# regicide211212/multi-style-transfer-gan

Hardware: AMD Instinct MI355X
Metric: train-step images/sec (fwd+bwd+loss), 256x256 batch32 (higher is better)
Workload: dtype f32; 1 GPU; config 3: reference CycleGAN train_step (2x EnhancedGenerator + 2x EnhancedDiscriminator, channels=16, num_transformer_blocks=0), 32 image pairs/GPU at 256x256, fwd+bwd+loss+Adam; per_gpu_batch=32, size=256, channels=16, parallelism=dp1, collective=none, losses_finite=True

## Files before the change

multi-style-transfer-gan_amd/mstg_hip/csrc/common.h:

```cpp
#pragma once
#include <hip/hip_runtime.h>
#include <stdint.h>
#include <stdio.h>
#include <string.h>

#include "mstg_hip.h"

typedef float f32x4 __attribute__((ext_vector_type(4)));
typedef float f32x2 __attribute__((ext_vector_type(2)));

namespace mstg {

extern thread_local char g_last_error[256];
inline int fail_launch(hipError_t e, const char* what) {
    snprintf(g_last_error, sizeof(g_last_error), "%s: %s", what, hipGetErrorString(e));
    return MSTG_E_LAUNCH;
}
inline int fail_arg(int code, const char* what) {
    snprintf(g_last_error, sizeof(g_last_error), "%s", what);
    return code;
}
#define MSTG_CHECK_LAUNCH(what)                                   \
    do {                                                          \
        hipError_t e__ = hipGetLastError();                       \
        if (e__ != hipSuccess) return mstg::fail_launch(e__, what); \
    } while (0)

extern bool g_prof_on;
void prof_begin(const void* host_fn, hipStream_t st);
void prof_end(hipStream_t st);
#define MSTG_LAUNCH(kern, grid, block, lds, st, ...)                               \
    do {                                                                           \
        const bool prof__ = mstg::g_prof_on;                                       \
        if (prof__) mstg::prof_begin((const void*)(kern), (hipStream_t)(st));      \
        hipLaunchKernelGGL(kern, grid, block, lds, st, __VA_ARGS__);               \
        if (prof__) mstg::prof_end((hipStream_t)(st));                             \
    } while (0)

extern thread_local bool t_ws_packed;
#define MSTG_PACK_LAUNCH(...)                      \
    do {                                           \
        if (!mstg::t_ws_packed) MSTG_LAUNCH(__VA_ARGS__); \
    } while (0)

enum EnvKnob {
    ENV_ATTN_BLK4, ENV_ATTN_BLK64, ENV_WGRAD_1X1, ENV_WGRAD_TS_MAXCH, ENV_WGRAD_PLAIN, ENV_WGRAD_OLD, ENV_NO_DPACK, ENV_IGEMM,
    ENV_STREAM, ENV_PF, ENV_WGLOB, ENV_HEAVY_PER_CU, ENV_DBG, ENV_DBG_LDS_KB, ENV_MS_WGRAD_PACKED, ENV_MS_FWD4, ENV_NO_PACK_CACHE,
    ENV_P32, ENV_P32_TH, ENV_P32_WLDS, ENV_P32_DBG, ENV_P32_OCC, ENV_ATTN_REG, ENV_NFW_ADAPT, ENV_BSUMS_ALL, ENV_ATTN_BIG32, ENV_NORM_WGS,
    ENV_CONV_IMG, ENV_COUNT
};
const char* env_get(EnvKnob k);

int cu_count();
struct OccCache {
    const void* kern = nullptr;
    size_t lds = 0;
    int occ = 1;
};
int persistent_occupancy(OccCache& c, const void* kern, size_t lds);

constexpr int WAVE = 64;

__device__ __forceinline__ f32x4 mfma16(float a, float b, f32x4 c) {
    return __builtin_amdgcn_mfma_f32_16x16x4f32(a, b, c, 0, 0, 0);
}

__device__ __forceinline__ float wave_sum(float v) {
#pragma unroll
    for (int o = 32; o > 0; o >>= 1) v += __shfl_xor(v, o, 64);
    return v;
}

__device__ __forceinline__ float apply_act(float v, int act) {
    switch (act) {
        case MSTG_ACT_RELU: return v > 0.f ? v : 0.f;
        case MSTG_ACT_LEAKY02: return v > 0.f ? v : 0.2f * v;
        case MSTG_ACT_TANH: return tanhf(v);
        case MSTG_ACT_GELU: return 0.5f * v * (1.f + erff(v * 0.70710678118654752f));
        default: return v;
    }
}
__device__ __forceinline__ float act_grad(float v, int act) {
    switch (act) {
        case MSTG_ACT_RELU: return v > 0.f ? 1.f : 0.f;
        case MSTG_ACT_LEAKY02: return v > 0.f ? 1.f : 0.2f;
        case MSTG_ACT_TANH: return 1.f - v * v;
        case MSTG_ACT_GELU: return 0.5f * (1.f + erff(v * 0.70710678118654752f)) + v * 0.3989422804014327f * expf(-0.5f * v * v);
        default: return 1.f;
    }
}

__device__ __forceinline__ int xcd_swizzle(int bid, int nblk) {
    const int q = nblk >> 3, r = nblk & 7, xcd = bid & 7, k = bid >> 3;
    return (xcd < r ? xcd * (q + 1) : r * (q + 1) + (xcd - r) * q) + k;
}


__host__ __device__ __forceinline__ unsigned magic_u32(unsigned d) { return 0xFFFFFFFFu / d + 1u; }

template <int NB>
__device__ __forceinline__ void stage_window_batch(const float* __restrict__ img, float* __restrict__ lds, int total, int e0, int cols,
                                                   int nq, unsigned m_cols, unsigned m_nq, int y0, int x0, int H, int W, int ctot,
                                                   int nq_valid, int ckp, int tid, int rowpad) {
    f32x4 v[NB];
    int dst[NB];
    bool ok[NB];
#pragma unroll
    for (int k = 0; k < NB; ++k) {
        const int e = e0 + 256 * k + tid;
        const int p = nq == 1 ? e : (int)__umulhi((unsigned)e, m_nq);
        const int q = e - p * nq;
        const int r = (int)__umulhi((unsigned)p, m_cols), c = p - r * cols;
        const int iy = y0 + r, ix = x0 + c;
        ok[k] = e < total && (unsigned)iy < (unsigned)H && (unsigned)ix < (unsigned)W && q < nq_valid;
        const unsigned off = ok[k] ? (unsigned)(iy * W + ix) * (unsigned)ctot + 4u * q : 0u;
        v[k] = *reinterpret_cast<const f32x4*>(img + off);
        dst[k] = e < total ? p * ckp + 4 * q + r * rowpad : -1;
    }
#pragma unroll
    for (int k = 0; k < NB; ++k)
        if (dst[k] >= 0) *reinterpret_cast<f32x4*>(&lds[dst[k]]) = ok[k] ? v[k] : f32x4{0.f, 0.f, 0.f, 0.f};
}

__device__ __forceinline__ void stage_window(const float* __restrict__ img, float* __restrict__ lds, int rows, int cols, int nq,
                                             unsigned m_cols, unsigned m_nq, int y0, int x0, int H, int W, int ctot, int nq_valid,
                                             int ckp, int tid, int rowpad = 0) {
    const int total = rows * cols * nq;
    int e0 = 0;
    for (; e0 + 1024 < total; e0 += 2048)
        stage_window_batch<8>(img, lds, total, e0, cols, nq, m_cols, m_nq, y0, x0, H, W, ctot, nq_valid, ckp, tid, rowpad);
    for (; e0 < total; e0 += 1024)
        stage_window_batch<4>(img, lds, total, e0, cols, nq, m_cols, m_nq, y0, x0, H, W, ctot, nq_valid, ckp, tid, rowpad);
}

__device__ __forceinline__ void stage_window_c4(const float* __restrict__ img, float* __restrict__ lds, int rows, int cols,
                                                unsigned m_cols, int y0, int x0, int H, int W, unsigned sy, unsigned sx, unsigned sc,
                                                int nch, int tid) {
    const int total = rows * cols;
    for (int e0 = 0; e0 < total; e0 += 1024) {
        f32x4 v[4];
        bool ok[4];
#pragma unroll
        for (int k = 0; k < 4; ++k) {
            const int e = e0 + 256 * k + tid;
            const int r = (int)__umulhi((unsigned)e, m_cols), c = e - r * cols;
            const int iy = y0 + r, ix = x0 + c;
            ok[k] = e < total && (unsigned)iy < (unsigned)H && (unsigned)ix < (unsigned)W;
            const unsigned off = ok[k] ? (unsigned)iy * sy + (unsigned)ix * sx : 0u;
#pragma unroll
            for (int ch = 0; ch < 4; ++ch) v[k][ch] = img[off + (ch < nch ? ch * sc : 0u)];
        }
#pragma unroll
        for (int k = 0; k < 4; ++k) {
            const int e = e0 + 256 * k + tid;
            if (e < total) {
                f32x4 w = {0.f, 0.f, 0.f, 0.f};
#pragma unroll
                for (int ch = 0; ch < 4; ++ch)
                    if (ok[k] && ch < nch) w[ch] = v[k][ch];
                *reinterpret_cast<f32x4*>(&lds[e * 4]) = w;
            }
        }
    }
}

inline int cdiv(int a, int b) { return (a + b - 1) / b; }
inline size_t cdivz(size_t a, size_t b) { return (a + b - 1) / b; }

}
```

multi-style-transfer-gan_amd/mstg_hip/csrc/norm.hip:

```cpp
#include "common.h"
#include <stdlib.h>

namespace mstg {

constexpr float NORM_EPS = 1e-5f;

struct NormGeom {
    int N, HW, C, split, chunk;
};

static NormGeom norm_geom(int N, int HW, int C) {
    NormGeom g;
    g.N = N; g.HW = HW; g.C = C;
    int wgs = 1024;
    { const char* e = env_get(ENV_NORM_WGS); if (e && atoi(e) >= 64) wgs = atoi(e); }
    int split = wgs / (N > 0 ? N : 1);
    if (split < 1) split = 1;
    const int maxsplit = cdiv(HW, 256);
    if (split > maxsplit) split = maxsplit;
    g.chunk = cdiv(HW, split);
    g.split = cdiv(HW, g.chunk);
    return g;
}

template <bool BWD>
__global__ __launch_bounds__(256) void norm_partial_kernel(const float* __restrict__ x, const float* __restrict__ dy,
                                                           const float* __restrict__ stats, const float* __restrict__ gamma,
                                                           const float* __restrict__ beta, float* __restrict__ partial,
                                                           NormGeom g, int act, int batch) {
    extern __shared__ __attribute__((aligned(16))) float red[];
    const int C = g.C, C4 = C >> 2, rows = 256 / C4;
    const int sp = blockIdx.x, n = blockIdx.y, tid = threadIdx.x;
    const int q = tid % C4, row = tid / C4;
    const int p0 = sp * g.chunk, p1 = min(g.HW, p0 + g.chunk);
    const float* xb = x + (size_t)n * g.HW * C;
    f32x4 s1 = {0.f, 0.f, 0.f, 0.f}, s2 = {0.f, 0.f, 0.f, 0.f};
    if (row < rows) {
        if (!BWD) {
            const f32x4 K = *reinterpret_cast<const f32x4*>((batch ? x : xb) + 4 * q);
            int p = p0 + row;
            constexpr int PX = 8;
            for (; p + (PX - 1) * rows < p1; p += PX * rows) {
                f32x4 v[PX];
#pragma unroll
                for (int k = 0; k < PX; ++k) v[k] = *reinterpret_cast<const f32x4*>(xb + (size_t)(p + k * rows) * C + 4 * q);
#pragma unroll
                for (int k = 0; k < PX; ++k) {
                    const f32x4 w = v[k] - K;
                    s1 += w;
                    s2 += w * w;
                }
            }
            for (; p < p1; p += rows) {
                const f32x4 v = *reinterpret_cast<const f32x4*>(xb + (size_t)p * C + 4 * q) - K;
                s1 += v;
                s2 += v * v;
            }
        } else {
            const float* st = stats + (size_t)(batch ? 0 : n) * C * 2;
            f32x4 mu, rs, ga = {1.f, 1.f, 1.f, 1.f}, be = {0.f, 0.f, 0.f, 0.f};
#pragma unroll
            for (int e = 0; e < 4; ++e) { mu[e] = st[(4 * q + e) * 2]; rs[e] = st[(4 * q + e) * 2 + 1]; }
            if (batch) { ga = *reinterpret_cast<const f32x4*>(gamma + 4 * q); be = *reinterpret_cast<const f32x4*>(beta + 4 * q); }
            const float* dyb = dy + (size_t)n * g.HW * C;
            int p = p0 + row;
            constexpr int PX = 8;
            for (; p + (PX - 1) * rows < p1; p += PX * rows) {
                f32x4 xv[PX], gv[PX];
#pragma unroll
                for (int k = 0; k < PX; ++k) {
                    xv[k] = *reinterpret_cast<const f32x4*>(xb + (size_t)(p + k * rows) * C + 4 * q);
                    gv[k] = *reinterpret_cast<const f32x4*>(dyb + (size_t)(p + k * rows) * C + 4 * q);
                }
#pragma unroll
                for (int k = 0; k < PX; ++k) {
                    const f32x4 xh = (xv[k] - mu) * rs;
                    f32x4 gg = gv[k];
#pragma unroll
                    for (int e = 0; e < 4; ++e) gg[e] *= act_grad(xh[e] * ga[e] + be[e], act);
                    s1 += gg;
                    s2 += gg * xh;
                }
            }
            for (; p < p1; p += rows) {
                const f32x4 xh = (*reinterpret_cast<const f32x4*>(xb + (size_t)p * C + 4 * q) - mu) * rs;
                f32x4 gg = *reinterpret_cast<const f32x4*>(dyb + (size_t)p * C + 4 * q);
#pragma unroll
                for (int e = 0; e < 4; ++e) gg[e] *= act_grad(xh[e] * ga[e] + be[e], act);
                s1 += gg;
                s2 += gg * xh;
            }
        }
        *reinterpret_cast<f32x4*>(&red[(row * 2 + 0) * C + 4 * q]) = s1;
        *reinterpret_cast<f32x4*>(&red[(row * 2 + 1) * C + 4 * q]) = s2;
    }
    __syncthreads();
    for (int e = tid; e < 2 * C; e += 256) {
        float acc = 0.f;
        for (int r = 0; r < rows; ++r) acc += red[r * 2 * C + e];
        partial[((size_t)n * g.split + sp) * 2 * C + e] = acc;
    }
}

template <bool BWD>
__global__ __launch_bounds__(256) void norm_apply_kernel(const float* __restrict__ x, const float* __restrict__ dy,
                                                         const float* __restrict__ residual, float* __restrict__ out,
                                                         float* __restrict__ stats, const float* __restrict__ gamma,
                                                         const float* __restrict__ beta, float* __restrict__ running_mean,
                                                         float* __restrict__ running_var, float* __restrict__ dgamma,
                                                         float* __restrict__ dbeta, const float* __restrict__ partial,
                                                         NormGeom g, int act, int batch, int psplit) {
    extern __shared__ __attribute__((aligned(16))) float sm[];
    const int C = g.C, C4 = C >> 2, rows = 256 / C4;
    const int sp = blockIdx.x, n = blockIdx.y, tid = threadIdx.x;
    const float cnt = batch ? (float)g.N * (float)g.HW : (float)g.HW;
    for (int c = tid; c < C; c += 256) {
        float t1 = 0.f, t2 = 0.f;
        if (batch != 2 && batch != 3) {
            const int nb = batch ? 0 : n, ne = batch ? g.N : n + 1;
            for (int nn = nb; nn < ne; ++nn) {
                const float* pp = partial + (size_t)nn * psplit * 2 * C + c;
                int s = 0;
                for (; s + 8 <= psplit; s += 8) {
                    float a[8], b[8];
#pragma unroll
                    for (int k = 0; k < 8; ++k) {
                        a[k] = pp[(size_t)(s + k) * 2 * C];
                        b[k] = pp[(size_t)(s + k) * 2 * C + C];
                    }
#pragma unroll
                    for (int k = 0; k < 8; ++k) {
                        t1 += a[k];
                        t2 += b[k];
                    }
                }
                for (; s < psplit; ++s) {
                    t1 += pp[(size_t)s * 2 * C];
                    t2 += pp[(size_t)s * 2 * C + C];
                }
            }
        }
        if (!BWD) {
            float mean, rstd;
            if (batch == 2) {
                mean = running_mean[c];
                rstd = rsqrtf(running_var[c] + NORM_EPS);
            } else if (batch == 3) {
                mean = stats[((size_t)n * C + c) * 2];
                rstd = stats[((size_t)n * C + c) * 2 + 1];
            } else {
                const float K = (batch ? x : x + (size_t)n * g.HW * C)[c];
                const float e1 = t1 / cnt;
                float var = t2 / cnt - e1 * e1;
                var = var > 0.f ? var : 0.f;
                mean = K + e1;
                rstd = rsqrtf(var + NORM_EPS);
                if (batch == 1 && sp == 0 && n == 0) {
                    running_mean[c] = 0.9f * running_mean[c] + 0.1f * mean;
                    running_var[c] = 0.9f * running_var[c] + 0.1f * var * (cnt / fmaxf(cnt - 1.f, 1.f));
                }
            }
            if (batch != 3 && sp == 0 && (!batch || n == 0)) {
                stats[((size_t)(batch ? 0 : n) * C + c) * 2] = mean;
                stats[((size_t)(batch ? 0 : n) * C + c) * 2 + 1] = rstd;
            }
            const bool affine = batch == 1 || batch == 2;
            const float ga = affine ? gamma[c] : 1.f, be = affine ? beta[c] : 0.f;
            sm[c] = rstd * ga;
            sm[C + c] = be;
            sm[2 * C + c] = mean;
        } else {
            const float* st = stats + (size_t)(batch ? 0 : n) * C * 2;
            const float mu = st[c * 2], rs = st[c * 2 + 1];
            const float ga = batch ? gamma[c] : 1.f;
            const float m1 = batch == 2 ? 0.f : t1 / cnt, m2 = batch == 2 ? 0.f : t2 / cnt;
            if (batch == 1 && sp == 0 && n == 0) { dgamma[c] = t2; dbeta[c] = t1; }
            sm[c] = mu;
            sm[C + c] = rs;
            sm[2 * C + c] = m1;
            sm[3 * C + c] = m2;
            (void)ga;
        }
    }
    __syncthreads();
    const int q = tid % C4, row = tid / C4;
    if (row >= rows) return;
    const int p0 = sp * g.chunk, p1 = min(g.HW, p0 + g.chunk);
    const size_t base = (size_t)n * g.HW * C;
    if (!BWD) {
        const f32x4 A = *reinterpret_cast<const f32x4*>(&sm[4 * q]), B = *reinterpret_cast<const f32x4*>(&sm[C + 4 * q]);
        const f32x4 M = *reinterpret_cast<const f32x4*>(&sm[2 * C + 4 * q]);
        int p = p0 + row;
        constexpr int PX = 8;
        for (; p + (PX - 1) * rows < p1; p += PX * rows) {
            f32x4 v[PX], r[PX];
#pragma unroll
            for (int k = 0; k < PX; ++k) {
                const size_t o = base + (size_t)(p + k * rows) * C + 4 * q;
                v[k] = __builtin_nontemporal_load(reinterpret_cast<const f32x4*>(x + o));
                if (residual) r[k] = __builtin_nontemporal_load(reinterpret_cast<const f32x4*>(residual + o));
            }
#pragma unroll
            for (int k = 0; k < PX; ++k) {
                const size_t o = base + (size_t)(p + k * rows) * C + 4 * q;
                f32x4 w = (v[k] - M) * A + B;
#pragma unroll
                for (int e = 0; e < 4; ++e) w[e] = apply_act(w[e], act);
                if (residual) w += r[k];
                *reinterpret_cast<f32x4*>(out + o) = w;
            }
        }
        for (; p < p1; p += rows) {
            const size_t o = base + (size_t)p * C + 4 * q;
            f32x4 v = (*reinterpret_cast<const f32x4*>(x + o) - M) * A + B;
#pragma unroll
            for (int e = 0; e < 4; ++e) v[e] = apply_act(v[e], act);
            if (residual) v += *reinterpret_cast<const f32x4*>(residual + o);
            *reinterpret_cast<f32x4*>(out + o) = v;
        }
    } else {
        const f32x4 mu = *reinterpret_cast<const f32x4*>(&sm[4 * q]), rs = *reinterpret_cast<const f32x4*>(&sm[C + 4 * q]);
        const f32x4 m1 = *reinterpret_cast<const f32x4*>(&sm[2 * C + 4 * q]), m2 = *reinterpret_cast<const f32x4*>(&sm[3 * C + 4 * q]);
        f32x4 ga = {1.f, 1.f, 1.f, 1.f}, be = {0.f, 0.f, 0.f, 0.f};
        if (batch) { ga = *reinterpret_cast<const f32x4*>(gamma + 4 * q); be = *reinterpret_cast<const f32x4*>(beta + 4 * q); }
        int p = p0 + row;
        constexpr int PX = 8;
        for (; p + (PX - 1) * rows < p1; p += PX * rows) {
            f32x4 xv[PX], gv[PX];
#pragma unroll
            for (int k = 0; k < PX; ++k) {
                const size_t o = base + (size_t)(p + k * rows) * C + 4 * q;
                xv[k] = __builtin_nontemporal_load(reinterpret_cast<const f32x4*>(x + o));
                gv[k] = __builtin_nontemporal_load(reinterpret_cast<const f32x4*>(dy + o));
            }
#pragma unroll
            for (int k = 0; k < PX; ++k) {
                const size_t o = base + (size_t)(p + k * rows) * C + 4 * q;
                const f32x4 xh = (xv[k] - mu) * rs;
                f32x4 gg = gv[k];
#pragma unroll
                for (int e = 0; e < 4; ++e) gg[e] *= act_grad(xh[e] * ga[e] + be[e], act);
                *reinterpret_cast<f32x4*>(out + o) = rs * ga * (gg - m1 - xh * m2);
            }
        }
        for (; p < p1; p += rows) {
            const size_t o = base + (size_t)p * C + 4 * q;
            const f32x4 xh = (*reinterpret_cast<const f32x4*>(x + o) - mu) * rs;
            f32x4 gg = *reinterpret_cast<const f32x4*>(dy + o);
#pragma unroll
            for (int e = 0; e < 4; ++e) gg[e] *= act_grad(xh[e] * ga[e] + be[e], act);
            *reinterpret_cast<f32x4*>(out + o) = rs * ga * (gg - m1 - xh * m2);
        }
    }
}

__device__ __forceinline__ void norm_row_sums(const float* __restrict__ partial, int n, int split, int C, int groups, float* red, float& t1,
                                              float& t2) {
    const int tid = threadIdx.x, c = tid % C, grp = tid / C;
    t1 = t2 = 0.f;
    if (grp < groups) {
        const float* pp = partial + (size_t)n * split * 2 * C + c;
        int s = grp;
        for (; s + 7 * groups < split; s += 8 * groups) {
            float a[8], b[8];
#pragma unroll
            for (int k = 0; k < 8; ++k) {
                a[k] = pp[(size_t)(s + k * groups) * 2 * C];
                b[k] = pp[(size_t)(s + k * groups) * 2 * C + C];
            }
#pragma unroll
            for (int k = 0; k < 8; ++k) {
                t1 += a[k];
                t2 += b[k];
            }
        }
        for (; s < split; s += groups) {
            t1 += pp[(size_t)s * 2 * C];
            t2 += pp[(size_t)s * 2 * C + C];
        }
    }
    if (groups > 1) {
        if (grp < groups) {
            red[(grp * 2 + 0) * C + c] = t1;
            red[(grp * 2 + 1) * C + c] = t2;
        }
        __syncthreads();
        if (grp == 0) {
            t1 = t2 = 0.f;
            for (int k = 0; k < groups; ++k) {
                t1 += red[(k * 2 + 0) * C + c];
                t2 += red[(k * 2 + 1) * C + c];
            }
        }
    }
}

static int norm_groups(const NormGeom& g) { return g.split > 32 && g.C <= 128 ? 256 / g.C : 1; }
static int norm_row_threads(const NormGeom& g) { const int t = g.C * norm_groups(g); return t < 64 ? 64 : ((t + 63) / 64) * 64; }

__global__ void norm_stats_kernel(const float* __restrict__ x, const float* __restrict__ partial, float* __restrict__ stats, NormGeom g,
                                  int groups) {
    extern __shared__ __attribute__((aligned(16))) float red[];
    const int n = blockIdx.x, C = g.C;
    const float cnt = (float)g.HW;
    float t1, t2;
    norm_row_sums(partial, n, g.split, C, groups, red, t1, t2);
    if ((int)threadIdx.x < C) {
        const int c = threadIdx.x;
        const float K = x[(size_t)n * g.HW * C + c];
        const float e1 = t1 / cnt;
        float var = t2 / cnt - e1 * e1;
        var = var > 0.f ? var : 0.f;
        stats[((size_t)n * C + c) * 2] = K + e1;
        stats[((size_t)n * C + c) * 2 + 1] = rsqrtf(var + NORM_EPS);
    }
}

__global__ void norm_sums_kernel(const float* __restrict__ partial, float* __restrict__ sums, NormGeom g, int groups) {
    extern __shared__ __attribute__((aligned(16))) float red[];
    const int n = blockIdx.x, C = g.C;
    float t1, t2;
    norm_row_sums(partial, n, g.split, C, groups, red, t1, t2);
    if ((int)threadIdx.x < C) {
        sums[((size_t)n * 2 + 0) * C + threadIdx.x] = t1;
        sums[((size_t)n * 2 + 1) * C + threadIdx.x] = t2;
    }
}

static int norm_check(int N, int HW, int C) {
    if (N <= 0 || HW <= 0 || C <= 0) return fail_arg(MSTG_E_BADARG, "norm: empty tensor");
    if (C % 4 || C > 1024) return fail_arg(MSTG_E_ALIGN, "norm: C must be a multiple of 4 and <= 1024");
    return MSTG_OK;
}

}

using namespace mstg;

extern "C" size_t mstg_norm_workspace_bytes(int N, int HW, int C) {
    if (N <= 0 || HW <= 0 || C <= 0) return 0;
    const NormGeom g = norm_geom(N, HW, C);
    return ((size_t)N * g.split * 2 * C + (size_t)N * 2 * C) * sizeof(float);
}

extern "C" int mstg_norm_act_fwd(const float* x, const float* residual, float* y, float* stats, int N, int HW, int C, int act,
                                 int batch_stats, const float* gamma, const float* beta, float* running_mean,
                                 float* running_var, void* workspace, size_t workspace_bytes, void* stream) {
    if (int rc = norm_check(N, HW, C)) return rc;
    if (!x || !y || !stats || !workspace) return fail_arg(MSTG_E_BADARG, "norm_fwd: null pointer");
    if (batch_stats && (!gamma || !beta || !running_mean || !running_var)) return fail_arg(MSTG_E_BADARG, "norm_fwd: batch norm needs gamma/beta/running stats");
    if (act == MSTG_ACT_TANH) return fail_arg(MSTG_E_UNSUPPORTED, "norm_fwd: tanh epilogue not supported");
    const NormGeom g = norm_geom(N, HW, C);
    if (workspace_bytes < mstg_norm_workspace_bytes(N, HW, C)) return fail_arg(MSTG_E_WORKSPACE, "norm_fwd: workspace too small");
    hipStream_t st = (hipStream_t)stream;
    const int rows = 256 / (C / 4);
    dim3 grid(g.split, N);
    if (batch_stats != 2) {
        MSTG_LAUNCH((norm_partial_kernel<false>), grid, dim3(256), (size_t)rows * 2 * C * sizeof(float), st, x, nullptr, nullptr,
                           gamma, beta, (float*)workspace, g, act, batch_stats);
        MSTG_CHECK_LAUNCH("norm_partial_kernel");
    }
    if (batch_stats == 0 && g.split > 32) {
        const int groups = norm_groups(g);
        MSTG_LAUNCH(norm_stats_kernel, dim3(N), dim3(norm_row_threads(g)), (size_t)groups * 2 * C * sizeof(float), st, x,
                    (const float*)workspace, stats, g, groups);
        MSTG_CHECK_LAUNCH("norm_stats_kernel");
        MSTG_LAUNCH((norm_apply_kernel<false>), grid, dim3(256), (size_t)4 * C * sizeof(float), st, x, nullptr, residual, y, stats, nullptr,
                    nullptr, nullptr, nullptr, nullptr, nullptr, nullptr, g, act, 3, 0);
        MSTG_CHECK_LAUNCH("norm_apply_kernel");
        return MSTG_OK;
    }
    MSTG_LAUNCH((norm_apply_kernel<false>), grid, dim3(256), (size_t)4 * C * sizeof(float), st, x, nullptr, residual, y, stats,
                       gamma, beta, running_mean, running_var, nullptr, nullptr, (const float*)workspace, g, act, batch_stats, g.split);
    MSTG_CHECK_LAUNCH("norm_apply_kernel");
    return MSTG_OK;
}

extern "C" int mstg_norm_act_bwd(const float* x, const float* stats, const float* dy, float* dx, int N, int HW, int C, int act,
                                 int batch_stats, const float* gamma, const float* beta, float* dgamma, float* dbeta,
                                 void* workspace, size_t workspace_bytes, void* stream) {
    if (int rc = norm_check(N, HW, C)) return rc;
    if (!x || !stats || !dy || !dx || !workspace) return fail_arg(MSTG_E_BADARG, "norm_bwd: null pointer");
    if (batch_stats == 1 && (!gamma || !beta || !dgamma || !dbeta)) return fail_arg(MSTG_E_BADARG, "norm_bwd: batch norm needs gamma/beta/dgamma/dbeta");
    if (batch_stats == 2) return fail_arg(MSTG_E_UNSUPPORTED, "norm_bwd: eval-mode batch norm backward not implemented");
    const NormGeom g = norm_geom(N, HW, C);
    if (workspace_bytes < mstg_norm_workspace_bytes(N, HW, C)) return fail_arg(MSTG_E_WORKSPACE, "norm_bwd: workspace too small");
    hipStream_t st = (hipStream_t)stream;
    const int rows = 256 / (C / 4);
    dim3 grid(g.split, N);
    MSTG_LAUNCH((norm_partial_kernel<true>), grid, dim3(256), (size_t)rows * 2 * C * sizeof(float), st, x, dy, stats, gamma, beta,
                       (float*)workspace, g, act, batch_stats);
    MSTG_CHECK_LAUNCH("norm_partial_kernel<bwd>");
    if (batch_stats == 0 && g.split > 32) {
        const int groups = norm_groups(g);
        float* sums = (float*)workspace + (size_t)N * g.split * 2 * C;
        MSTG_LAUNCH(norm_sums_kernel, dim3(N), dim3(norm_row_threads(g)), (size_t)groups * 2 * C * sizeof(float), st, (const float*)workspace,
                    sums, g, groups);
        MSTG_CHECK_LAUNCH("norm_sums_kernel");
        MSTG_LAUNCH((norm_apply_kernel<true>), grid, dim3(256), (size_t)4 * C * sizeof(float), st, x, dy, nullptr, dx, const_cast<float*>(stats),
                    gamma, beta, nullptr, nullptr, dgamma, dbeta, (const float*)sums, g, act, batch_stats, 1);
        MSTG_CHECK_LAUNCH("norm_apply_kernel<bwd>");
        return MSTG_OK;
    }
    MSTG_LAUNCH((norm_apply_kernel<true>), grid, dim3(256), (size_t)4 * C * sizeof(float), st, x, dy, nullptr, dx,
                       const_cast<float*>(stats), gamma, beta, nullptr, nullptr, dgamma, dbeta, (const float*)workspace, g, act,
                       batch_stats, g.split);
    MSTG_CHECK_LAUNCH("norm_apply_kernel<bwd>");
    return MSTG_OK;
}

extern "C" int mstg_norm_stats(const float* x, float* stats, int N, int HW, int C, void* workspace, size_t workspace_bytes,
                               void* stream) {
    if (int rc = norm_check(N, HW, C)) return rc;
    if (!x || !stats || !workspace) return fail_arg(MSTG_E_BADARG, "norm_stats: null pointer");
    const NormGeom g = norm_geom(N, HW, C);
    if (workspace_bytes < mstg_norm_workspace_bytes(N, HW, C)) return fail_arg(MSTG_E_WORKSPACE, "norm_stats: workspace too small");
    hipStream_t st = (hipStream_t)stream;
    const int rows = 256 / (C / 4);
    MSTG_LAUNCH((norm_partial_kernel<false>), dim3(g.split, N), dim3(256), (size_t)rows * 2 * C * sizeof(float), st, x, nullptr,
                       nullptr, nullptr, nullptr, (float*)workspace, g, MSTG_ACT_NONE, 0);
    MSTG_CHECK_LAUNCH("norm_partial_kernel");
    const int groups = norm_groups(g);
    MSTG_LAUNCH(norm_stats_kernel, dim3(N), dim3(norm_row_threads(g)), (size_t)groups * 2 * C * sizeof(float), st, x, (const float*)workspace,
                stats, g, groups);
    MSTG_CHECK_LAUNCH("norm_stats_kernel");
    return MSTG_OK;
}

extern "C" int mstg_norm_bwd_apply(const float* x, const float* stats, const float* dy, const float* sums, int sums_split, float* dx,
                                   int N, int HW, int C, int act, void* stream) {
    if (int rc = norm_check(N, HW, C)) return rc;
    if (!x || !stats || !dy || !sums || !dx) return fail_arg(MSTG_E_BADARG, "norm_bwd_apply: null pointer");
    if (sums_split < 1) return fail_arg(MSTG_E_BADARG, "norm_bwd_apply: sums_split must be >= 1");
    const NormGeom g = norm_geom(N, HW, C);
    MSTG_LAUNCH((norm_apply_kernel<true>), dim3(g.split, N), dim3(256), (size_t)4 * C * sizeof(float), (hipStream_t)stream, x, dy,
                       nullptr, dx, const_cast<float*>(stats), nullptr, nullptr, nullptr, nullptr, nullptr, nullptr, sums, g, act, 0, sums_split);
    MSTG_CHECK_LAUNCH("norm_apply_kernel<bwd>");
    return MSTG_OK;
}

extern "C" int mstg_norm_apply_fwd(const float* x, const float* stats, const float* residual, float* y, int N, int HW, int C, int act,
                                   void* stream) {
    if (int rc = norm_check(N, HW, C)) return rc;
    if (!x || !stats || !y) return fail_arg(MSTG_E_BADARG, "norm_apply_fwd: null pointer");
    if (act == MSTG_ACT_TANH) return fail_arg(MSTG_E_UNSUPPORTED, "norm_apply_fwd: tanh epilogue not supported");
    const NormGeom g = norm_geom(N, HW, C);
    MSTG_LAUNCH((norm_apply_kernel<false>), dim3(g.split, N), dim3(256), (size_t)4 * C * sizeof(float), (hipStream_t)stream, x, nullptr,
                       residual, y, const_cast<float*>(stats), nullptr, nullptr, nullptr, nullptr, nullptr, nullptr, nullptr, g, act, 3, 0);
    MSTG_CHECK_LAUNCH("norm_apply_kernel");
    return MSTG_OK;
}
```

multi-style-transfer-gan_amd/mstg_hip/csrc/runtime.hip:

```cpp
#include <stdlib.h>

#include <cxxabi.h>

#include <mutex>
#include <string>
#include <vector>

#include "common.h"

namespace mstg {

thread_local char g_last_error[256] = "";
thread_local bool t_ws_packed = false;

static const char* const kEnvNames[ENV_COUNT] = {
    "MSTG_ATTN_BLK4", "MSTG_ATTN_BLK64", "MSTG_WGRAD_1X1", "MSTG_WGRAD_TS_MAXCH", "MSTG_WGRAD_PLAIN", "MSTG_WGRAD_OLD", "MSTG_NO_DPACK",
    "MSTG_IGEMM", "MSTG_STREAM", "MSTG_PF", "MSTG_WGLOB", "MSTG_HEAVY_PER_CU", "MSTG_DBG", "MSTG_DBG_LDS_KB", "MSTG_MS_WGRAD_PACKED",
    "MSTG_MS_FWD4", "MSTG_NO_PACK_CACHE", "MSTG_P32", "MSTG_P32_TH", "MSTG_P32_WLDS", "MSTG_P32_DBG", "MSTG_P32_OCC", "MSTG_ATTN_REG", "MSTG_NFW_ADAPT", "MSTG_BSUMS_ALL", "MSTG_ATTN_BIG32", "MSTG_NORM_WGS",
    "MSTG_CONV_IMG"};

struct EnvCache {
    char val[ENV_COUNT][32];
    bool set[ENV_COUNT];
    EnvCache() { refresh(); }
    void refresh() {
        for (int k = 0; k < ENV_COUNT; ++k) {
            const char* e = getenv(kEnvNames[k]);
            set[k] = e != nullptr;
            snprintf(val[k], sizeof(val[k]), "%s", e ? e : "");
        }
    }
};
static EnvCache g_env;

const char* env_get(EnvKnob k) { return g_env.set[k] ? g_env.val[k] : nullptr; }

int cu_count() {
    static int cus = 0;
    if (!cus) {
        int dev = 0;
        hipDeviceProp_t p;
        if (hipGetDevice(&dev) == hipSuccess && hipGetDeviceProperties(&p, dev) == hipSuccess) cus = p.multiProcessorCount;
        if (cus <= 0) cus = 256;
    }
    return cus;
}

int persistent_occupancy(OccCache& c, const void* kern, size_t lds) {
    if (c.kern != kern || c.lds != lds) {
        if (lds > 64 * 1024) (void)hipFuncSetAttribute(kern, hipFuncAttributeMaxDynamicSharedMemorySize, 160 * 1024);
        int nb = 1;
        if (hipOccupancyMaxActiveBlocksPerMultiprocessor(&nb, kern, 256, lds) != hipSuccess || nb < 1) nb = 1;
        c.occ = nb > 4 ? 4 : nb;
        c.kern = kern;
        c.lds = lds;
    }
    return c.occ;
}

bool g_prof_on = false;
struct ProfRec {
    const void* fn;
    hipStream_t st;
    hipEvent_t e0, e1;
};
static std::vector<ProfRec> g_prof;
static std::mutex g_prof_mu;
static thread_local int t_prof_open = -1;

void prof_begin(const void* fn, hipStream_t st) {
    ProfRec r{fn, st, nullptr, nullptr};
    if (hipEventCreate(&r.e0) != hipSuccess || hipEventCreate(&r.e1) != hipSuccess) return;
    (void)hipEventRecord(r.e0, st);
    std::lock_guard<std::mutex> lk(g_prof_mu);
    t_prof_open = (int)g_prof.size();
    g_prof.push_back(r);
}
void prof_end(hipStream_t st) {
    std::lock_guard<std::mutex> lk(g_prof_mu);
    if (t_prof_open < 0 || t_prof_open >= (int)g_prof.size()) return;
    (void)hipEventRecord(g_prof[t_prof_open].e1, st);
    t_prof_open = -1;
}
static void prof_clear() {
    for (auto& r : g_prof) {
        (void)hipEventDestroy(r.e0);
        (void)hipEventDestroy(r.e1);
    }
    g_prof.clear();
}

}

extern "C" const char* mstg_version(void) { return "mstg-hip 0.2.0 gfx950"; }
extern "C" const char* mstg_arch(void) { return "gfx950"; }
extern "C" const char* mstg_last_error(void) { return mstg::g_last_error; }
extern "C" void mstg_env_refresh(void) { mstg::g_env.refresh(); }

extern "C" int mstg_prof_enable(int on) {
    std::lock_guard<std::mutex> lk(mstg::g_prof_mu);
    if (on) mstg::prof_clear();
    mstg::g_prof_on = on != 0;
    return MSTG_OK;
}
extern "C" int mstg_prof_count(void) {
    std::lock_guard<std::mutex> lk(mstg::g_prof_mu);
    return (int)mstg::g_prof.size();
}
extern "C" int mstg_prof_get(int i, char* name, size_t name_cap, float* ms) {
    mstg::ProfRec r;
    {
        std::lock_guard<std::mutex> lk(mstg::g_prof_mu);
        if (i < 0 || i >= (int)mstg::g_prof.size() || !name || !ms || name_cap < 8) return mstg::fail_arg(MSTG_E_BADARG, "mstg_prof_get: bad index or buffer");
        r = mstg::g_prof[i];
    }
    hipError_t e = hipEventSynchronize(r.e1);
    if (e == hipSuccess) e = hipEventElapsedTime(ms, r.e0, r.e1);
    if (e != hipSuccess) return mstg::fail_launch(e, "mstg_prof_get");
    const char* mangled = hipKernelNameRefByPtr(r.fn, r.st);
    std::string nm = mangled ? mangled : "?";
    int status = 0;
    char* dem = mangled ? abi::__cxa_demangle(mangled, nullptr, nullptr, &status) : nullptr;
    if (dem && status == 0) nm = dem;
    free(dem);
    int depth = 0, cut = -1;
    for (int k = (int)nm.size() - 1; k >= 0; --k) {
        if (nm[k] == ')') ++depth;
        else if (nm[k] == '(' && --depth == 0) { cut = k; break; }
    }
    if (cut > 0) nm.resize(cut);
    if (nm.rfind("void ", 0) == 0) nm.erase(0, 5);
    if (nm.rfind("mstg::", 0) == 0) nm.erase(0, 6);
    snprintf(name, name_cap, "%s", nm.c_str());
    return MSTG_OK;
}
```

Measured before the change: 1715 images/sec.

## Add single-kernel per-plane instance norm fwd/bwd for small spatial sizes

Adds fused instance-norm forward and backward kernels for small planes (HW<=1024, leaky-ReLU, no residual, no batch stats). One workgroup owns an (image, 4-channel) plane, stages it in LDS, computes the ordered sums and then normalizes and applies the activation in the same launch. This replaces the multi-kernel partial-reduce/apply path, aiming to cut launch count and extra global traffic for the small, deep layers. The cost is that each block handles only 4 channels, so global loads are strided by C and occupancy is limited by LDS. The path is on by default and can be disabled with an env knob.

Result: no change. 1728 images/sec (median of 6 runs) (+0.7%).

```diff
diff --git a/multi-style-transfer-gan_amd/mstg_hip/csrc/common.h b/multi-style-transfer-gan_amd/mstg_hip/csrc/common.h
--- a/multi-style-transfer-gan_amd/mstg_hip/csrc/common.h
+++ b/multi-style-transfer-gan_amd/mstg_hip/csrc/common.h
@@ -47,7 +47,7 @@
     ENV_ATTN_BLK4, ENV_ATTN_BLK64, ENV_WGRAD_1X1, ENV_WGRAD_TS_MAXCH, ENV_WGRAD_PLAIN, ENV_WGRAD_OLD, ENV_NO_DPACK, ENV_IGEMM,
     ENV_STREAM, ENV_PF, ENV_WGLOB, ENV_HEAVY_PER_CU, ENV_DBG, ENV_DBG_LDS_KB, ENV_MS_WGRAD_PACKED, ENV_MS_FWD4, ENV_NO_PACK_CACHE,
     ENV_P32, ENV_P32_TH, ENV_P32_WLDS, ENV_P32_DBG, ENV_P32_OCC, ENV_ATTN_REG, ENV_NFW_ADAPT, ENV_BSUMS_ALL, ENV_ATTN_BIG32, ENV_NORM_WGS,
-    ENV_CONV_IMG, ENV_COUNT
+    ENV_CONV_IMG, ENV_NORM_PLANE, ENV_COUNT
 };
 const char* env_get(EnvKnob k);
 
diff --git a/multi-style-transfer-gan_amd/mstg_hip/csrc/norm.hip b/multi-style-transfer-gan_amd/mstg_hip/csrc/norm.hip
--- a/multi-style-transfer-gan_amd/mstg_hip/csrc/norm.hip
+++ b/multi-style-transfer-gan_amd/mstg_hip/csrc/norm.hip
@@ -327,6 +327,162 @@
     }
 }
 
+constexpr int PLANE_MAX_HW = 1024;
+
+static bool norm_plane_on() {
+    const char* e = env_get(ENV_NORM_PLANE);
+    return !(e && e[0] == '0');
+}
+static bool norm_plane_ok(const NormGeom& g, int act, int batch_stats, const float* residual) {
+    return norm_plane_on() && batch_stats == 0 && !residual && g.HW <= PLANE_MAX_HW && act == MSTG_ACT_LEAKY02 &&
+           g.split * (256 / (g.C / 4)) <= 256;
+}
+static int norm_plane_grid(int N, int C) { return 8 * (C / 4) * cdiv(N, 8); }
+
+__device__ __forceinline__ bool plane_owner(int N, int C4, int& n, int& q) {
+    const int b = blockIdx.x, k = b >> 3;
+    q = k % C4;
+    n = (k / C4) * 8 + (b & 7);
+    return n < N;
+}
+
+template <bool BWD>
+__device__ __forceinline__ void plane_ordered_sums(const f32x4* xs, const f32x4* gs, f32x4 K, const NormGeom& g, int rows, int act, float* red,
+                                                   float* part, f32x4& t1, f32x4& t2) {
+    const int tid = threadIdx.x;
+    if (tid < g.split * rows) {
+        const int sp = tid / rows, row = tid - sp * rows;
+        const int p0 = sp * g.chunk, p1 = min(g.HW, p0 + g.chunk);
+        f32x4 s1 = {0.f, 0.f, 0.f, 0.f}, s2 = {0.f, 0.f, 0.f, 0.f};
+        for (int p = p0 + row; p < p1; p += rows) {
+            if (!BWD) {
+                const f32x4 w = xs[p] - K;
+                s1 += w;
+                s2 += w * w;
+            } else {
+                const f32x4 xh = xs[p];
+                f32x4 gg = gs[p];
+#pragma unroll
+                for (int e = 0; e < 4; ++e) gg[e] *= act_grad(xh[e], act);
+                s1 += gg;
+                s2 += gg * xh;
+            }
+        }
+        *reinterpret_cast<f32x4*>(&red[tid * 8]) = s1;
+        *reinterpret_cast<f32x4*>(&red[tid * 8 + 4]) = s2;
+    }
+    __syncthreads();
+    if (tid < 8 * g.split) {
+        const int sp = tid >> 3, e = tid & 7;
+        float acc = 0.f;
+        for (int r = 0; r < rows; ++r) acc += red[(sp * rows + r) * 8 + e];
+        part[tid] = acc;
+    }
+    __syncthreads();
+    t1 = t2 = f32x4{0.f, 0.f, 0.f, 0.f};
+    for (int s = 0; s < g.split; ++s) {
+        t1 += *reinterpret_cast<const f32x4*>(&part[s * 8]);
+        t2 += *reinterpret_cast<const f32x4*>(&part[s * 8 + 4]);
+    }
+}
+
+template <int PX>
+__global__ __launch_bounds__(256) void norm_plane_fwd_kernel(const float* __restrict__ x, float* __restrict__ y, float* __restrict__ stats,
+                                                             NormGeom g, int act) {
+    __shared__ f32x4 xs[256 * PX];
+    __shared__ __attribute__((aligned(16))) float red[256 * 8];
+    __shared__ __attribute__((aligned(16))) float part[4 * 8];
+    const int C = g.C, HW = g.HW;
+    int n, q;
+    if (!plane_owner(g.N, C >> 2, n, q)) return;
+    const int tid = threadIdx.x;
+    const size_t base = (size_t)n * HW * C + 4 * q;
+    const f32x4 K = *reinterpret_cast<const f32x4*>(x + base);
+    f32x4 v[PX];
+#pragma unroll
+    for (int k = 0; k < PX; ++k) {
+        const int p = tid + 256 * k;
+        if (p < HW) {
+            v[k] = *reinterpret_cast<const f32x4*>(x + base + (size_t)p * C);
+            xs[p] = v[k];
+        }
+    }
+    __syncthreads();
+    f32x4 t1, t2;
+    plane_ordered_sums<false>(xs, nullptr, K, g, 256 / (C >> 2), act, red, part, t1, t2);
+    const float cnt = (float)HW;
+    f32x4 M, A;
+    const f32x4 B = {0.f, 0.f, 0.f, 0.f};
+#pragma unroll
+    for (int e = 0; e < 4; ++e) {
+        const float e1 = t1[e] / cnt;
+        float var = t2[e] / cnt - e1 * e1;
+        var = var > 0.f ? var : 0.f;
+        M[e] = K[e] + e1;
+        A[e] = rsqrtf(var + NORM_EPS);
+    }
+    if (tid == 0) {
+        float* st = stats + ((size_t)n * C + 4 * q) * 2;
+#pragma unroll
+        for (int e = 0; e < 4; ++e) { st[2 * e] = M[e]; st[2 * e + 1] = A[e]; }
+    }
+#pragma unroll
+    for (int k = 0; k < PX; ++k) {
+        const int p = tid + 256 * k;
+        if (p < HW) {
+            f32x4 w = (v[k] - M) * A + B;
+#pragma unroll
+            for (int e = 0; e < 4; ++e) w[e] = apply_act(w[e], act);
+            *reinterpret_cast<f32x4*>(y + base + (size_t)p * C) = w;
+        }
+    }
+}
+
+template <int PX>
+__global__ __launch_bounds__(256) void norm_plane_bwd_kernel(const float* __restrict__ x, const float* __restrict__ dy,
+                                                             const float* __restrict__ stats, float* __restrict__ dx, NormGeom g, int act) {
+    __shared__ f32x4 xs[256 * PX];
+    __shared__ f32x4 gs[256 * PX];
+    __shared__ __attribute__((aligned(16))) float red[256 * 8];
+    __shared__ __attribute__((aligned(16))) float part[4 * 8];
+    const int C = g.C, HW = g.HW;
+    int n, q;
+    if (!plane_owner(g.N, C >> 2, n, q)) return;
+    const int tid = threadIdx.x;
+    const size_t base = (size_t)n * HW * C + 4 * q;
+    const float* st = stats + ((size_t)n * C + 4 * q) * 2;
+    f32x4 mu, rs;
+    const f32x4 ga = {1.f, 1.f, 1.f, 1.f}, be = {0.f, 0.f, 0.f, 0.f};
+#pragma unroll
+    for (int e = 0; e < 4; ++e) { mu[e] = st[2 * e]; rs[e] = st[2 * e + 1]; }
+    f32x4 xh[PX], gv[PX];
+#pragma unroll
+    for (int k = 0; k < PX; ++k) {
+        const int p = tid + 256 * k;
+        if (p < HW) {
+            xh[k] = (*reinterpret_cast<const f32x4*>(x + base + (size_t)p * C) - mu) * rs;
+            gv[k] = *reinterpret_cast<const f32x4*>(dy + base + (size_t)p * C);
+            xs[p] = xh[k];
+            gs[p] = gv[k];
+        }
+    }
+    __syncthreads();
+    f32x4 t1, t2;
+    plane_ordered_sums<true>(xs, gs, mu, g, 256 / (C >> 2), act, red, part, t1, t2);
+    const float cnt = (float)HW;
+    const f32x4 m1 = t1 / cnt, m2 = t2 / cnt;
+#pragma unroll
+    for (int k = 0; k < PX; ++k) {
+        const int p = tid + 256 * k;
+        if (p < HW) {
+            f32x4 gg = gv[k];
+#pragma unroll
+            for (int e = 0; e < 4; ++e) gg[e] *= act_grad(xh[k][e] * ga[e] + be[e], act);
+            *reinterpret_cast<f32x4*>(dx + base + (size_t)p * C) = rs * ga * (gg - m1 - xh[k] * m2);
+        }
+    }
+}
+
 static int norm_check(int N, int HW, int C) {
     if (N <= 0 || HW <= 0 || C <= 0) return fail_arg(MSTG_E_BADARG, "norm: empty tensor");
     if (C % 4 || C > 1024) return fail_arg(MSTG_E_ALIGN, "norm: C must be a multiple of 4 and <= 1024");
@@ -353,6 +509,13 @@
     const NormGeom g = norm_geom(N, HW, C);
     if (workspace_bytes < mstg_norm_workspace_bytes(N, HW, C)) return fail_arg(MSTG_E_WORKSPACE, "norm_fwd: workspace too small");
     hipStream_t st = (hipStream_t)stream;
+    if (norm_plane_ok(g, act, batch_stats, residual)) {
+        const dim3 pgrid(norm_plane_grid(N, C));
+        if (HW <= 256) MSTG_LAUNCH(norm_plane_fwd_kernel<1>, pgrid, dim3(256), 0, st, x, y, stats, g, act);
+        else MSTG_LAUNCH(norm_plane_fwd_kernel<4>, pgrid, dim3(256), 0, st, x, y, stats, g, act);
+        MSTG_CHECK_LAUNCH("norm_plane_fwd_kernel");
+        return MSTG_OK;
+    }
     const int rows = 256 / (C / 4);
     dim3 grid(g.split, N);
     if (batch_stats != 2) {
@@ -386,6 +549,13 @@
     const NormGeom g = norm_geom(N, HW, C);
     if (workspace_bytes < mstg_norm_workspace_bytes(N, HW, C)) return fail_arg(MSTG_E_WORKSPACE, "norm_bwd: workspace too small");
     hipStream_t st = (hipStream_t)stream;
+    if (norm_plane_ok(g, act, batch_stats, nullptr)) {
+        const dim3 pgrid(norm_plane_grid(N, C));
+        if (HW <= 256) MSTG_LAUNCH(norm_plane_bwd_kernel<1>, pgrid, dim3(256), 0, st, x, dy, stats, dx, g, act);
+        else MSTG_LAUNCH(norm_plane_bwd_kernel<4>, pgrid, dim3(256), 0, st, x, dy, stats, dx, g, act);
+        MSTG_CHECK_LAUNCH("norm_plane_bwd_kernel");
+        return MSTG_OK;
+    }
     const int rows = 256 / (C / 4);
     dim3 grid(g.split, N);
     MSTG_LAUNCH((norm_partial_kernel<true>), grid, dim3(256), (size_t)rows * 2 * C * sizeof(float), st, x, dy, stats, gamma, beta,
diff --git a/multi-style-transfer-gan_amd/mstg_hip/csrc/runtime.hip b/multi-style-transfer-gan_amd/mstg_hip/csrc/runtime.hip
--- a/multi-style-transfer-gan_amd/mstg_hip/csrc/runtime.hip
+++ b/multi-style-transfer-gan_amd/mstg_hip/csrc/runtime.hip
@@ -17,7 +17,7 @@
     "MSTG_ATTN_BLK4", "MSTG_ATTN_BLK64", "MSTG_WGRAD_1X1", "MSTG_WGRAD_TS_MAXCH", "MSTG_WGRAD_PLAIN", "MSTG_WGRAD_OLD", "MSTG_NO_DPACK",
     "MSTG_IGEMM", "MSTG_STREAM", "MSTG_PF", "MSTG_WGLOB", "MSTG_HEAVY_PER_CU", "MSTG_DBG", "MSTG_DBG_LDS_KB", "MSTG_MS_WGRAD_PACKED",
     "MSTG_MS_FWD4", "MSTG_NO_PACK_CACHE", "MSTG_P32", "MSTG_P32_TH", "MSTG_P32_WLDS", "MSTG_P32_DBG", "MSTG_P32_OCC", "MSTG_ATTN_REG", "MSTG_NFW_ADAPT", "MSTG_BSUMS_ALL", "MSTG_ATTN_BIG32", "MSTG_NORM_WGS",
-    "MSTG_CONV_IMG"};
+    "MSTG_CONV_IMG", "MSTG_NORM_PLANE"};
 
 struct EnvCache {
     char val[ENV_COUNT][32];
```
